# ChaissonLab/LRA

Hardware: AMD Instinct MI355X
Metric: aligned Gbp/s, 30 kb ONT vs GRCh38 (MapRead_lowacc end to end incl. SAM text), per job (higher is better)
Workload: dtype int32

## Files before the change

### lra_amd/csrc/indel_refine.hip

```cpp
#include "common.h"
#include "scan.h"
#include <algorithm>
#include <stdlib.h>

int lra_aog_launch_device(lra_ctx* ctx, int n, const char* d_qseq, const char* d_tseq, const uint64_t* d_q_off,
                          const int32_t* d_q_len, const uint64_t* d_t_off, const int32_t* d_t_len, const int32_t* d_k,
                          int m, int mm, int indel, int32_t* d_score, int32_t* d_nblocks, int32_t* d_blocks,
                          const uint64_t* d_block_off, int32_t* d_status);

namespace {

constexpr int BAD = -999999999;
constexpr int NEG = -2000000000;
enum { C_DIAG = 0, C_LEFT = 1, C_DOWN = 2, C_BOUND = 3, C_DELCLOSE = 4, C_INSCLOSE = 5, C_DONE = 6 };

__device__ __forceinline__ void wave_sync() {
  __builtin_amdgcn_fence(__ATOMIC_RELEASE, "workgroup");
  __builtin_amdgcn_wave_barrier();
  __builtin_amdgcn_fence(__ATOMIC_ACQUIRE, "workgroup");
}

__device__ __forceinline__ void wave_sync_lds() {
  __builtin_amdgcn_fence(__ATOMIC_RELEASE, "wavefront");
  __builtin_amdgcn_wave_barrier();
// ... 283 lines not shown
        }
    }
    if (st.btGap > st.bqGap) {
      for (int ti = 0; ti < st.btGap; ti++) {
        if (tOff >= tLen) { status |= 1; break; }
        const int e = (int)min(qEnd - 1, q + k);
        RG(ringS, tOff) = (int)max(q - k, qStart); RG(ringE, tOff) = e;
        if (e < eMin) eMin = e;
        if (sHi < tOff) sHi = tOff;
        tOff++;
        flush(tOff - k);
      }
    }
    bq = nq2; bt = nt2; bl = nl2;
  }
  if (lastChunk) for (long r = max(0L, tOff - k + 1); r < tLen; r++) flush(r);
#undef RG
  if (!multi) { if (tOff != tLen) status |= 1; B.s_status[s] = status; }
}

__global__ void __launch_bounds__(64) ir_band_scan(BandArgs B) {
  const uint64_t s = blockIdx.x;
  const int lane = threadIdx.x;
  if (B.s_kind[s] != 0) { if (lane == 0) { B.s_cells[s] = 0; B.s_status[s] = 0; B.s_width[s] = 0; B.s_tmpcap[s] = 0; } return; }
  int status = B.s_status[s];
  const long tLen = (long)B.s_rows[s];
  Row* rows = B.rows + B.s_row_off[s];
  unsigned long long cells = 0;
  int width = 0;
  if (!status && tLen > 0) {
    int run = 0x7fffffff;
    for (long base = ((tLen - 1) / 64) * 64; base >= 0; base -= 64) {
      const long r = base + lane;
      const int own = (r < tLen) ? rows[r].S : 0x7fffffff;
      int v = own;
      for (int d = 1; d < 64; d <<= 1) { int o = __shfl_down(v, d); if (lane + d < 64) v = min(v, o); }
      v = min(v, run);
      if (r < tLen && v != own) rows[r].S = v;
      run = __shfl(v, 0);
    }
    const int a = B.s_aln[s];
    const unsigned char* tb = (const unsigned char*)B.tseq + B.t_off[a] + B.s_tStart[s];
    int runE = -0x7fffffff;
    for (long base = 0; base < tLen; base += 64) {
      const long r = base + lane;
      Row w; w.S = 0; w.E = -0x7fffffff; w.C = 0; w.T = 0;
      if (r < tLen) w = rows[r];
      int e = w.E;
      for (int d = 1; d < 64; d <<= 1) { int o = __shfl_up(e, d); if (lane >= d) e = max(e, o); }
      e = max(e, runE);
      runE = __shfl(e, 63);
      int len = (r < tLen) ? e - w.S + 1 : 0;
      if (r < tLen) {
        if (len < 1 || w.S < 0) status |= 1;
        else if (len > MAXW) status |= 4;
        width = max(width, len);
      }
      const unsigned long long l = (unsigned long long)max(len, 0);
      unsigned long long inc = l;
      for (int d = 1; d < 64; d <<= 1) { unsigned long long o = __shfl_up(inc, d); if (lane >= d) inc += o; }
      if (r < tLen) { w.E = e; w.C = (unsigned int)(cells + inc - l); w.T = tb[r]; rows[r] = w; }
      cells += __shfl(inc, 63);
    }
    for (int o = 32; o > 0; o >>= 1) { status |= __shfl_xor(status, o); width = max(width, __shfl_xor(width, o)); }
  }
  if (lane == 0) {
    B.s_cells[s] = status ? 0 : cells;
    B.s_status[s] = status;
    B.s_width[s] = status ? 0 : width;
    B.s_tmpcap[s] = status ? 0 : (uint64_t)(tLen + ((long)B.s_qEnd[s] - B.s_qStart[s]) + 2);
  }
}

constexpr int FILL_BINS = 128;
template <bool EMIT>
__global__ void ir_classify(uint64_t n_seg, const int32_t* __restrict__ s_kind, const int32_t* __restrict__ s_status, const int32_t* __restrict__ s_width,
                            const uint64_t* __restrict__ s_rows, int* bins, uint32_t* list) {
  const uint64_t s = (uint64_t)blockIdx.x * blockDim.x + threadIdx.x;
  const int lane = threadIdx.x & 63;
  int bin = -1;
  if (s < n_seg && s_kind[s] == 0 && s_status[s] == 0) {
    const int w = s_width[s];
    const uint32_t r = (uint32_t)min((unsigned long long)s_rows[s], 0x7fffffffULL);
    bin = (w <= 16 ? 0 : w <= 32 ? 1 : w <= 64 ? 2 : 3) * 32 + (r ? __clz(r) : 31);
  }
  const unsigned long long below = (lane == 0) ? 0ULL : (~0ULL >> (64 - lane));
  unsigned long long todo = __ballot(bin >= 0);
  while (todo) {
    const int leader = __ffsll((long long)todo) - 1;
    const int b = __shfl(bin, leader);
    const unsigned long long m = __ballot(bin == b);
    int base = 0;
    if (lane == leader) base = atomicAdd(&bins[b], __popcll(m));
    base = __shfl(base, leader);
    if (EMIT && bin == b) list[base + __popcll(m & below)] = (uint32_t)s;
    todo &= ~m;
  }
}

struct FillArgs {
  uint64_t n_seg;
  const int32_t* s_aln; const uint64_t* s_rows; const uint64_t* s_row_off; const uint64_t* s_cell_off;
  const Row* rows;
  const char* qseq; const uint64_t* q_off; const int32_t* q_len;
  int match, mismatch, g;
  unsigned char* path;
  const uint32_t* list; int* cursor;
};

__device__ __forceinline__ bool is_bound(long row, int c, int len) { return c == len - 1 || (row > 0 && c == 0); }

__device__ __forceinline__ int shr1(int x, int fill) { return __builtin_amdgcn_update_dpp(fill, x, 0x138, 0xf, 0xf, false); }
template <int G>
__device__ __forceinline__ int scan_max(int w) {
  w = max(w, __builtin_amdgcn_update_dpp(NEG, w, 0x111, 0xf, 0xf, false));
  w = max(w, __builtin_amdgcn_update_dpp(NEG, w, 0x112, 0xf, 0xf, false));
  w = max(w, __builtin_amdgcn_update_dpp(NEG, w, 0x114, 0xf, 0xf, false));
  w = max(w, __builtin_amdgcn_update_dpp(NEG, w, 0x118, 0xf, 0xf, false));
  if (G >= 32) w = max(w, __builtin_amdgcn_update_dpp(NEG, w, 0x142, 0xa, 0xf, false));
  if (G >= 64) w = max(w, __builtin_amdgcn_update_dpp(NEG, w, 0x143, 0xc, 0xf, false));
  return w;
}

template <int G>
__global__ void __launch_bounds__(64) ir_fill(FillArgs F) {
  constexpr int GP = 64 / G;
  constexpr int CLS = (G == 16) ? 0 : (G == 32) ? 1 : 2;
  const int lane = threadIdx.x;
  const int c = lane % G, gbase = lane - c;
  const int g = F.g, go = 2 * F.g + 1;
  const long listEnd = F.cursor[4 + CLS];
  const uint32_t* list = F.list;
  long ti = -1, tLen = 0;
  const Row* rows = nullptr; const unsigned char* qb = nullptr; unsigned char* P = nullptr;
  long chunkBase = 0, qLast = 0;
  Row chunk; chunk.S = chunk.E = chunk.T = 0; chunk.C = 0;
  int W0 = 0, qlo = 0, qhi = 0, qnext = 0;
  int prevM = BAD, prevD = BAD, prevS = 0, prevLen = 0;
  bool done = false;
  auto ldq = [&](long idx) -> int { return qb[idx < qLast ? idx : qLast]; };
  while (true) {
    if (!done && ti < 0) {
      long x = 0;
      if (c == 0) x = atomicAdd(&F.cursor[CLS], 1);
      x = __shfl(x, gbase);
      if (x < listEnd) {
        const uint64_t s = list[x];
        const int a = F.s_aln[s];
        tLen = (long)F.s_rows[s];
        rows = F.rows + F.s_row_off[s];
        qb = (const unsigned char*)F.qseq + F.q_off[a];
        qLast = (long)F.q_len[a] - 1;
        P = F.path + F.s_cell_off[s];
        ti = 0; chunkBase = 0;
        if (c < tLen) chunk = rows[c];
        W0 = rows[0].S;
        qlo = ldq((long)W0 + c); qhi = ldq((long)W0 + G + c); qnext = ldq((long)W0 + 2 * G + c);
      } else done = true;
    }
    if (__ballot(!done) == 0ULL) break;
    if (!done && ti - chunkBase == G) { chunkBase = ti; if (ti + c < tLen) chunk = rows[ti + c]; }
    const int src = gbase + (int)((ti - chunkBase) & (G - 1));
    const int S = __shfl(chunk.S, src), E = __shfl(chunk.E, src), tch = __shfl(chunk.T, src);
    const unsigned int C = __shfl(chunk.C, src);
    while (!done && S - W0 >= G) { W0 += G; qlo = qhi; qhi = qnext; qnext = ldq((long)W0 + 2 * G + c); }
    const int j = S - W0 + c;
    const int q1 = __shfl(qlo, gbase + (j & (G - 1))), q2 = __shfl(qhi, gbase + (j & (G - 1)));
    const int qch = (j < G) ? q1 : q2;
    const int len = E - S + 1;
    const bool lastRow = (ti == tLen - 1);
    const int off = S - prevS;
    const bool interior = c >= 1 && (lastRow ? c <= len - 1 : c <= len - 2);
    const int srcA = c + off, srcD = srcA - 1;
    const bool aboveIn = srcA <= prevLen - 1;
    const int aM = __shfl(prevM, gbase + (srcA & (G - 1))), aD = __shfl(prevD, gbase + (srcA & (G - 1)));
    const int dM = shr1(aM, BAD);
    const bool okA = aboveIn && !is_bound(ti - 1, srcA, prevLen);
    const bool okD = aboveIn && srcD >= 0 && !is_bound(ti - 1, srcD, prevLen);
    const int dOpen = okA ? aM + go : BAD, dExt = okA ? aD : BAD;
    const int Dv = max(dOpen, dExt);
    const int delOpen = (Dv == dOpen) ? 1 : 0;
    const int mS = okD ? dM + (tch == qch ? F.match : F.mismatch) : BAD;
    const int dS = okA ? aM + g : BAD;
    const int V = interior ? max(mS, max(dS, Dv)) : NEG;
    const int W = scan_max<G>(V);
    int Wm1 = shr1(W, NEG), Vm1 = shr1(V, NEG);
    if (c == 0) { Wm1 = NEG; Vm1 = NEG; }
    const int Iv = max(BAD, go + Wm1);
    int M = max(max(BAD, V), max(Vm1 + g, go + Wm1));
    if (!interior) M = BAD;
    int Mleft = shr1(M, BAD);
    if (c <= 1) Mleft = BAD;
    const int iOpen = Mleft + go;
    const int insOpen = (Iv == iOpen) ? 1 : 0;
    const int iS = Mleft + g;
    int code;
    if (!interior) code = C_BOUND;
    else if (M == mS) code = C_DIAG;
    else if (M == iS) code = C_LEFT;
    else if (M == dS) code = C_DOWN;
    else if (M == Dv) code = C_DELCLOSE;
    else code = C_INSCLOSE;
    int outM = M, outD = interior ? Dv : BAD;
    unsigned char outB = (unsigned char)(code | (delOpen << 3) | (insOpen << 4));
    if (ti == 0) {
      const bool last0 = (c == len - 1) && (tLen > 1);
      outM = last0 ? BAD : (c == 0 ? 0 : c * g);
      outD = BAD;
      outB = (unsigned char)(last0 ? C_BOUND : (c == 0 ? C_DONE : C_LEFT));
    }
    if (!done) {
      if (c < len) P[C + c] = outB;
      prevM = outM; prevD = outD; prevS = S; prevLen = len;
      ti++;
      if (ti == tLen) ti = -1;
    }
  }
}


__global__ void __launch_bounds__(64) ir_fill_wide(FillArgs F) {
  __shared__ int sM[2][MAXW + 64], sD[2][MAXW + 64];
  const int lane = threadIdx.x;
  const int g = F.g, go = 2 * F.g + 1;
  const long listEnd = F.cursor[4 + 3];
  while (true) {
    long x = 0;
    if (lane == 0) x = atomicAdd(&F.cursor[3], 1);
    x = (long)(((unsigned long long)(unsigned)__builtin_amdgcn_readfirstlane((int)((unsigned long long)x >> 32)) << 32) | (unsigned)__builtin_amdgcn_readfirstlane((int)(x & 0xffffffffL)));
    if (x >= listEnd) break;
    const uint64_t s = F.list[x];
    const int a = F.s_aln[s];
    const long tLen = (long)F.s_rows[s];
    const Row* rows = F.rows + F.s_row_off[s];
    const unsigned char* qb = (const unsigned char*)F.qseq + F.q_off[a];
    const long qLast = (long)F.q_len[a] - 1;
    unsigned char* P = F.path + F.s_cell_off[s];
    int prevS = 0, prevLen = 0;
    for (long ti = 0; ti < tLen; ti++) {
      const Row rw = rows[ti];
      const int S = rw.S, len = rw.E - rw.S + 1, tch = rw.T;
      const unsigned int C = rw.C;
      const bool lastRow = (ti == tLen - 1);
      const int off = S - prevS;
      const int cur = (int)(ti & 1), prv = cur ^ 1;
      int carryW = NEG, carryV = NEG, carryM = BAD;
      for (int base = 0; base < len; base += 64) {
        const int c = base + lane;
        int outM, outD; unsigned char outB;
        if (ti == 0) {
          const bool last0 = (c == len - 1) && (tLen > 1);
          outM = last0 ? BAD : (c == 0 ? 0 : c * g);
          outD = BAD;
          outB = (unsigned char)(last0 ? C_BOUND : (c == 0 ? C_DONE : C_LEFT));
        } else {
          const long qi = (long)S + c;
          const int qch = qb[qi < qLast ? qi : qLast];
          const bool interior = c >= 1 && (lastRow ? c <= len - 1 : c <= len - 2);
          const int srcA = c + off, srcD = srcA - 1;
          const bool aboveIn = srcA <= prevLen - 1;
          const bool inA = srcA >= 0 && srcA < prevLen, inD = srcD >= 0 && srcD < prevLen;
          const int aM = inA ? sM[prv][srcA] : BAD, aD = inA ? sD[prv][srcA] : BAD;
          const int dM = inD ? sM[prv][srcD] : BAD;
          const bool okA = aboveIn && !is_bound(ti - 1, srcA, prevLen);
          const bool okD = aboveIn && srcD >= 0 && !is_bound(ti - 1, srcD, prevLen);
          const int dOpen = okA ? aM + go : BAD, dExt = okA ? aD : BAD;
          const int Dv = max(dOpen, dExt);
          const int delOpen = (Dv == dOpen) ? 1 : 0;
          const int mS = okD ? dM + (tch == qch ? F.match : F.mismatch) : BAD;
          const int dS = okA ? aM + g : BAD;
          const int V = interior ? max(mS, max(dS, Dv)) : NEG;
          const int W = max(scan_max<64>(V), carryW);
          int Wm1 = shr1(W, NEG), Vm1 = shr1(V, NEG);
          if (lane == 0) { Wm1 = carryW; Vm1 = carryV; }
          if (c == 0) { Wm1 = NEG; Vm1 = NEG; }
          const int Iv = max(BAD, go + Wm1);
          int M = max(max(BAD, V), max(Vm1 + g, go + Wm1));
          if (!interior) M = BAD;
          int Mleft = shr1(M, BAD);
          if (lane == 0) Mleft = carryM;
          if (c <= 1) Mleft = BAD;
          const int iOpen = Mleft + go;
          const int insOpen = (Iv == iOpen) ? 1 : 0;
          const int iS = Mleft + g;
          int code;
          if (!interior) code = C_BOUND;
          else if (M == mS) code = C_DIAG;
          else if (M == iS) code = C_LEFT;
          else if (M == dS) code = C_DOWN;
          else if (M == Dv) code = C_DELCLOSE;
          else code = C_INSCLOSE;
          outM = M; outD = interior ? Dv : BAD;
          outB = (unsigned char)(code | (delOpen << 3) | (insOpen << 4));
          carryW = __shfl(W, 63); carryV = __shfl(V, 63); carryM = __shfl(M, 63);
        }
        if (c < len) { P[C + c] = outB; sM[cur][c] = outM; sD[cur][c] = outD; }
      }
      wave_sync_lds();
      prevS = S; prevLen = len;
    }
  }
}

__global__ void __launch_bounds__(64) ir_fill_16x2(FillArgs F) {
  constexpr int G = 16;
  const int lane = threadIdx.x;
  const int c = lane % G, gbase = lane - c;
  const int g = F.g, go = 2 * F.g + 1;
  const long listEnd = F.cursor[4 + 1];
  const uint32_t* list = F.list;
  long ti = -1, tLen = 0;
  const Row* rows = nullptr; const unsigned char* qb = nullptr; unsigned char* P = nullptr;
  long chunkBase = 0, qLast = 0;
  Row chunk; chunk.S = chunk.E = chunk.T = 0; chunk.C = 0;
  int W0 = 0, q0 = 0, q1 = 0, q2 = 0, q3 = 0;
  int pM[2] = {BAD, BAD}, pD[2] = {BAD, BAD}, prevS = 0, prevLen = 0;
  bool done = false;
  auto ldq = [&](long idx) -> int { return qb[idx < qLast ? idx : qLast]; };
  while (true) {
    if (!done && ti < 0) {
      long x = 0;
      if (c == 0) x = atomicAdd(&F.cursor[1], 1);
      x = __shfl(x, gbase);
      if (x < listEnd) {
        const uint64_t s = list[x];
        const int a = F.s_aln[s];
        tLen = (long)F.s_rows[s];
        rows = F.rows + F.s_row_off[s];
        qb = (const unsigned char*)F.qseq + F.q_off[a];
        qLast = (long)F.q_len[a] - 1;
        P = F.path + F.s_cell_off[s];
        ti = 0; chunkBase = 0;
        if (c < tLen) chunk = rows[c];
        W0 = rows[0].S;
        q0 = ldq((long)W0 + c); q1 = ldq((long)W0 + G + c); q2 = ldq((long)W0 + 2 * G + c); q3 = ldq((long)W0 + 3 * G + c);
      } else done = true;
    }
    if (__ballot(!done) == 0ULL) break;
    if (!done && ti - chunkBase == G) { chunkBase = ti; if (ti + c < tLen) chunk = rows[ti + c]; }
    const int src = gbase + (int)((ti - chunkBase) & (G - 1));
    const int S = __shfl(chunk.S, src), E = __shfl(chunk.E, src), tch = __shfl(chunk.T, src);
    const unsigned int C = __shfl(chunk.C, src);
    while (!done && S - W0 >= G) { W0 += G; q0 = q1; q1 = q2; q2 = q3; q3 = ldq((long)W0 + 3 * G + c); }
    const int len = E - S + 1;
    const bool lastRow = (ti == tLen - 1);
    const int off = S - prevS;
    int nM[2] = {BAD, BAD}, nD[2] = {BAD, BAD};
    int carryW = NEG, carryV = NEG, carryM = BAD;
    const int np = (!done && len > G) ? 2 : 1;
    for (int p = 0; p < np; p++) {
      const int cc = c + G * p;
      const int j = S - W0 + cc;
      const int l = gbase + (j & (G - 1));
      const int qa = __shfl(q0, l), qbb = __shfl(q1, l), qc = __shfl(q2, l), qd = __shfl(q3, l);
      const int qch = (j < G) ? qa : (j < 2 * G) ? qbb : (j < 3 * G) ? qc : qd;
      const bool interior = cc >= 1 && (lastRow ? cc <= len - 1 : cc <= len - 2);
      const int srcA = cc + off, srcD = srcA - 1;
      const bool aboveIn = srcA <= prevLen - 1;
      const int la = gbase + (srcA & (G - 1)), ld = gbase + (srcD & (G - 1));
      const int a0 = __shfl(pM[0], la), a1 = __shfl(pM[1], la), b0 = __shfl(pD[0], la), b1 = __shfl(pD[1], la);
      const int d0 = __shfl(pM[0], ld), d1 = __shfl(pM[1], ld);
      const int aM = (srcA & G) ? a1 : a0, aD = (srcA & G) ? b1 : b0;
      const int dM = (srcD & G) ? d1 : d0;
      const bool okA = aboveIn && !is_bound(ti - 1, srcA, prevLen);
      const bool okD = aboveIn && srcD >= 0 && !is_bound(ti - 1, srcD, prevLen);
      const int dOpen = okA ? aM + go : BAD, dExt = okA ? aD : BAD;
      const int Dv = max(dOpen, dExt);
      const int delOpen = (Dv == dOpen) ? 1 : 0;
      const int mS = okD ? dM + (tch == qch ? F.match : F.mismatch) : BAD;
      const int dS = okA ? aM + g : BAD;
      const int V = interior ? max(mS, max(dS, Dv)) : NEG;
      const int W = max(scan_max<G>(V), carryW);
      int Wm1 = shr1(W, NEG), Vm1 = shr1(V, NEG);
      if (c == 0) { Wm1 = carryW; Vm1 = carryV; }
      const int Iv = max(BAD, go + Wm1);
      int M = max(max(BAD, V), max(Vm1 + g, go + Wm1));
      if (!interior) M = BAD;
      int Mleft = shr1(M, BAD);
      if (c == 0) Mleft = carryM;
      if (cc <= 1) Mleft = BAD;
      const int iOpen = Mleft + go;
      const int insOpen = (Iv == iOpen) ? 1 : 0;
      const int iS = Mleft + g;
      int code;
      if (!interior) code = C_BOUND;
      else if (M == mS) code = C_DIAG;
      else if (M == iS) code = C_LEFT;
      else if (M == dS) code = C_DOWN;
      else if (M == Dv) code = C_DELCLOSE;
      else code = C_INSCLOSE;
      int outM = M, outD = interior ? Dv : BAD;
      unsigned char outB = (unsigned char)(code | (delOpen << 3) | (insOpen << 4));
      if (ti == 0) {
        const bool last0 = (cc == len - 1) && (tLen > 1);
        outM = last0 ? BAD : (cc == 0 ? 0 : cc * g);
        outD = BAD;
        outB = (unsigned char)(last0 ? C_BOUND : (cc == 0 ? C_DONE : C_LEFT));
      }
      if (!done && cc < len) P[C + cc] = outB;
      nM[p] = outM; nD[p] = outD;
      carryW = __shfl(W, gbase + G - 1); carryV = __shfl(V, gbase + G - 1); carryM = __shfl(M, gbase + G - 1);
    }
    if (!done) {
      pM[0] = nM[0]; pM[1] = nM[1]; pD[0] = nD[0]; pD[1] = nD[1]; prevS = S; prevLen = len;
      ti++;
      if (ti == tLen) ti = -1;
    }
  }
}

struct TraceArgs {
  uint64_t n_seg;
  const int32_t* s_kind; const int32_t* s_tStart; const uint64_t* s_rows; const uint64_t* s_row_off;
  const uint64_t* s_cells; const uint64_t* s_cell_off; int32_t* s_status;
  const Row* rows;
  const unsigned char* path;
  uint32_t* s_nblk;
  const uint64_t* s_tmp_off; int32_t* tmp_blocks;
};

constexpr int TW_ROWS = 128, TW_PATH = 4096;
__global__ void __launch_bounds__(64) ir_trace_wave(TraceArgs T) {
  __shared__ Row s_rows[TW_ROWS];
  __shared__ __attribute__((aligned(16))) unsigned char s_path[TW_PATH + 16];
  const int lane = threadIdx.x;
  const uint64_t s = blockIdx.x;
  if (s >= T.n_seg) return;
  if (T.s_kind[s] != 0) return;
  if (T.s_status[s] != 0) { if (lane == 0) T.s_nblk[s] = 0; return; }
  const long tLen = (long)T.s_rows[s];
  const Row* rows = T.rows + T.s_row_off[s];
  const unsigned char* P = T.path + T.s_cell_off[s];
  int32_t* ob = T.tmp_blocks + 3 * T.s_tmp_off[s];
  const long cap = (long)(T.s_tmp_off[s + 1] - T.s_tmp_off[s]);
  long ti = tLen - 1;
  long rBase = 0, wLo = 1, wHi = 0; unsigned pBase = 0;
  auto stage = [&](long at) {
    wave_sync();
    wHi = at; rBase = max(0L, at - TW_ROWS + 1);
    for (long x = lane; x <= at - rBase; x += 64) s_rows[x] = rows[rBase + x];
    wave_sync();
    const Row last = s_rows[at - rBase];
    const unsigned end = last.C + (unsigned)max(last.E - last.S + 1, 0);
    long lo = rBase, hi = at;
    while (lo < hi) { const long mid = (lo + hi) >> 1; if (end - s_rows[mid - rBase].C <= (unsigned)TW_PATH) hi = mid; else lo = mid + 1; }
    wLo = lo; pBase = s_rows[lo - rBase].C;
    const unsigned nbytes = min(end - pBase, (unsigned)TW_PATH);
    const unsigned char* start = P + pBase;
    const unsigned delta = (unsigned)((uintptr_t)start & 15);
    const uint4* a16 = (const uint4*)(start - delta);
    const unsigned full = (delta + nbytes) >> 4;
    for (unsigned x = lane; x < full; x += 64) ((uint4*)s_path)[x] = a16[x];
    for (unsigned x = (full << 4) + lane; x < delta + nbytes; x += 64) s_path[x] = (start - delta)[x];
    pBase -= delta;
    wave_sync();
  };
  stage(ti);
  Row rw = s_rows[ti - rBase];
  int qa = rw.E;
  int mat = 0;
  int bad = 0;
  long nblk = 0;
  long q = (long)rw.E + 1, t = (long)T.s_tStart[s] + tLen;
  int curKind = -1, pending = 0;
  long dlen = 0;
  long steps = 0;
  const long step_cap = 4 * (long)T.s_cells[s] + 64;
  auto emit_block = [&]() {
    if (nblk < cap) { if (lane == 0) { ob[3 * nblk] = (int)q; ob[3 * nblk + 1] = (int)t; ob[3 * nblk + 2] = (int)dlen; } } else bad = 1;
    nblk++;
  };
  auto op = [&](int kind, long times) {
    if (kind != curKind) {
      if (curKind == -1 && kind == 0) { pending = 1; dlen = 0; }
      if (kind != 0) {
        if (pending) emit_block();
        pending = 1; dlen = 0;
      }
      curKind = kind;
    }
    if (kind == 0) { dlen += times; q -= times; t -= times; }
    else if (kind == 1) q -= times;
    else t -= times;
  };
  while (true) {
    if (ti < wLo || ti > wHi) stage(ti);
    rw = s_rows[ti - rBase];
    if (mat == 0) {
      const long tl = ti - lane;
      bool fast = false;
      if (tl >= wLo && tl >= 1) {
        const Row r = s_rows[tl - rBase];
        const int c = (qa - lane) - r.S;
        if (c >= 0 && c <= r.E - r.S) fast = (s_path[r.C - pBase + (unsigned)c] & 7) == C_DIAG;
      }
      const unsigned long long nf = ~__ballot(fast);
      const int f = nf ? __ffsll((long long)nf) - 1 : 64;
      if (f > 0) {
        steps += f;
        if (steps > step_cap) { bad = 1; break; }
        op(0, f); ti -= f; qa -= f;
        continue;
      }
    }
    const int c = qa - rw.S;
    if (c < 0 || c > rw.E - rw.S) { bad = 1; break; }
    if (ti == 0 && c == 0) break;
    if (++steps > step_cap) { bad = 1; break; }
    const unsigned char pb = s_path[rw.C - pBase + (unsigned)c];
    long nti = ti;
    if (mat == 0) {
      const int code = pb & 7;
      if (code == C_DELCLOSE) mat = 1;
      else if (code == C_INSCLOSE) mat = 2;
      else if (code == C_DIAG) { op(0, 1); nti = ti - 1; qa--; }
      else if (code == C_LEFT) { op(1, 1); qa--; }
      else if (code == C_DOWN) { op(2, 1); nti = ti - 1; }
      else { bad = 1; break; }
    } else if (mat == 1) {
      op(2, 1);
      mat = ((pb >> 3) & 1) ? 0 : 1;
      nti = ti - 1;
    } else {
      op(1, 1);
      mat = ((pb >> 4) & 1) ? 0 : 2;
      qa--;
    }
    if (nti != ti) {
      if (nti < 0) { bad = 1; break; }
      ti = nti;
    }
  }
  if (!bad) {
    op(0, 1);
    if (pending) emit_block();
  }
  if (lane == 0) {
    if (bad) T.s_status[s] |= 2;
    T.s_nblk[s] = bad ? 0 : (uint32_t)nblk;
  }
}

struct GatherArgs {
  uint64_t n_item;
  const int32_t* i_kind; const int32_t* i_data; const int32_t* i_aln; const uint64_t* i_out_off;
  const uint64_t* seg_off;
  const int32_t* s_kind; const int32_t* s_qStart; const int32_t* s_tStart; const uint32_t* s_aog_idx;
  const int32_t* aog_blocks; const uint64_t* aog_block_off; const int32_t* aog_nblocks;
  const int32_t* tmp_blocks; const uint64_t* s_tmp_off; const uint32_t* s_nblk;
  int32_t* out_blocks;
};

__global__ void ir_item_counts(uint64_t n_item, const int32_t* i_kind, const int32_t* i_data, const int32_t* i_aln, const uint64_t* seg_off,
                               const int32_t* s_kind, const uint32_t* s_nblk, const uint32_t* s_aog_idx, const int32_t* aog_nblocks,
                               uint32_t* i_count) {
  uint64_t i = (uint64_t)blockIdx.x * blockDim.x + threadIdx.x;
  if (i >= n_item) return;
  if (i_kind[i] == 0) { i_count[i] = 1; return; }
  uint64_t s = seg_off[i_aln[i]] + (uint64_t)i_data[3 * i];
  i_count[i] = (s_kind[s] == 0) ? s_nblk[s] : (uint32_t)aog_nblocks[s_aog_idx[s]];
}

__global__ void __launch_bounds__(64) ir_gather(GatherArgs G) {
  const int lane = threadIdx.x;
  for (uint64_t i = blockIdx.x; i < G.n_item; i += gridDim.x) {
    int32_t* out = G.out_blocks + 3 * G.i_out_off[i];
    if (G.i_kind[i] == 0) {
      if (lane < 3) out[lane] = G.i_data[3 * i + lane];
      continue;
    }
    uint64_t s = G.seg_off[G.i_aln[i]] + (uint64_t)G.i_data[3 * i];
    if (G.s_kind[s] == 0) {
      const int32_t* src = G.tmp_blocks + 3 * G.s_tmp_off[s];
      const int n = (int)G.s_nblk[s];
      for (int x = lane; x < n; x += 64) {
        const int y = n - 1 - x;
        out[3 * x] = src[3 * y]; out[3 * x + 1] = src[3 * y + 1]; out[3 * x + 2] = src[3 * y + 2];
      }
      continue;
    }
    const uint32_t p = G.s_aog_idx[s];
    const int32_t* src = G.aog_blocks + 3 * G.aog_block_off[p];
    const int n = G.aog_nblocks[p];
    const int qs = G.s_qStart[s], ts = G.s_tStart[s];
    for (int x = lane; x < n; x += 64) {
      out[3 * x] = src[3 * x] + qs; out[3 * x + 1] = src[3 * x + 1] + ts; out[3 * x + 2] = src[3 * x + 2];
    }
  }
}

__global__ void ir_finalize_offsets(int n_aln, uint64_t n_item, const uint64_t* item_off, const uint64_t* i_out_off, const int32_t* i_kind,
                                    const int32_t* i_data, const int32_t* i_aln, const uint64_t* seg_off, uint64_t* s_out_off,
                                    uint64_t* out_block_off) {
  uint64_t i = (uint64_t)blockIdx.x * blockDim.x + threadIdx.x;
  if (i <= (uint64_t)n_aln) out_block_off[i] = i_out_off[i < (uint64_t)n_aln ? item_off[i] : n_item];
  if (i < n_item && i_kind[i] == 1) s_out_off[seg_off[i_aln[i]] + (uint64_t)i_data[3 * i]] = i_out_off[i];
}

__global__ void ir_aln_status(int n_aln, const uint64_t* seg_off, const int32_t* s_kind, const int32_t* s_status, const uint32_t* s_aog_idx,
                              const int32_t* p_status, int32_t* a_status) {
  int a = blockIdx.x * blockDim.x + threadIdx.x;
  if (a >= n_aln) return;
  int st = 0;
  for (uint64_t s = seg_off[a]; s < seg_off[a + 1]; s++) {
    if (s_kind[s] == 0) { int x = s_status[s]; if (x & 1) st |= LRA_ST_OOB_SLOT; if (x & 2) st |= LRA_ST_NO_TERMINATION; if (x & 4) st |= LRA_ST_RANGE; }
    else st |= p_status[s_aog_idx[s]];
  }
  a_status[a] = st;
}

__global__ void ir_item_aln(int n_aln, const uint64_t* item_off, int32_t* i_aln) {
  int a = blockIdx.x * blockDim.x + threadIdx.x;
  if (a >= n_aln) return;
  for (uint64_t i = item_off[a]; i < item_off[a + 1]; i++) i_aln[i] = a;
}

__global__ void ir_aog_setup(uint64_t n_seg, const int32_t* s_kind, const int32_t* s_aln, const uint64_t* s_aog_off ,
                             const int32_t* s_qStart, const int32_t* s_tStart, const int32_t* s_qEnd, const int32_t* s_tEnd,
                             const uint64_t* q_off, const uint64_t* t_off, int k, uint32_t* s_aog_idx, uint64_t* p_q_off, int32_t* p_q_len,
                             uint64_t* p_t_off, int32_t* p_t_len, int32_t* p_k, uint32_t* p_cap) {
  uint64_t s = (uint64_t)blockIdx.x * blockDim.x + threadIdx.x;
  if (s >= n_seg) return;
  if (s_kind[s] != 1) { s_aog_idx[s] = 0; return; }
  uint32_t p = (uint32_t)s_aog_off[s];
  s_aog_idx[s] = p;
  int a = s_aln[s];
  p_q_off[p] = q_off[a] + (uint64_t)s_qStart[s]; p_q_len[p] = s_qEnd[s] - s_qStart[s];
  p_t_off[p] = t_off[a] + (uint64_t)s_tStart[s]; p_t_len[p] = s_tEnd[s] - s_tStart[s];
  p_k[p] = k;
  p_cap[p] = (uint32_t)(min(p_q_len[p], p_t_len[p]) + 1);
}


struct Arena {
  char* base; size_t cap, used;
  template <typename T> T* get(size_t n) {
    size_t bytes = (n * sizeof(T) + 255) & ~(size_t)255;
    if (used + bytes > cap) return nullptr;
    T* p = (T*)(base + used);
    used += bytes;
    return p;
  }
};

}

template <typename CT>
static void scan(lra_ctx* ctx, long n, const CT* c, uint64_t* off) {
  (void)lra_exclusive_scan<CT>(ctx, n, c, off);
}

static int d2h(lra_ctx* ctx, void* dst, const void* src, size_t bytes) {
  LRA_HIP_CHECK(ctx, hipMemcpyAsync(dst, src, bytes, hipMemcpyDeviceToHost, ctx->stream));
  LRA_HIP_CHECK(ctx, hipStreamSynchronize(ctx->stream));
  return LRA_OK;
}

extern "C" int lra_indel_refine_batch(lra_ctx* ctx, int n_aln, const int32_t* d_blocks_in, const uint64_t* d_block_off, uint64_t n_blocks_in,
                                      const char* d_qseq, const uint64_t* d_q_off, const int32_t* d_q_len, const char* d_tseq,
                                      const uint64_t* d_t_off, const int64_t* d_t_len, int refine_band, int match, int mismatch,
                                      int indel, int end_align, lra_refine_result* out) {
  if (!ctx || !out || n_aln < 0) return LRA_ERR_INVALID;
  if (refine_band < 2 || refine_band > 64) return lra_set_err(ctx, LRA_ERR_INVALID, "refine_band must be 2..64");
  if (indel >= 0) return lra_set_err(ctx, LRA_ERR_INVALID, "indel score must be negative");
  memset(out, 0, sizeof(*out));
  if (n_aln == 0) return LRA_OK;
  LRA_HIP_CHECK(ctx, hipSetDevice(ctx->device));
  hipStream_t st = ctx->stream;
  const size_t nA = (size_t)n_aln, nBk = (size_t)n_blocks_in + 2 * nA;
  const size_t perAln = ((nA * 4 + 255) & ~(size_t)255) * 3 + (((nA + 1) * 8 + 255) & ~(size_t)255) * 3;
  char* baseP = (char*)lra_ensure(ctx, 70, perAln + 4096);
  if (!baseP) return LRA_ERR_NOMEM;
  Arena ap{baseP, perAln + 4096, 0};
  IRArgs A;
  memset(&A, 0, sizeof A);
  A.n_aln = n_aln; A.blocks_in = d_blocks_in; A.block_off = d_block_off;
  A.qseq = d_qseq; A.q_off = d_q_off; A.q_len = d_q_len; A.tseq = d_tseq; A.t_off = d_t_off; A.t_len = d_t_len;
  A.k = refine_band; A.match = match; A.mismatch = mismatch; A.indel = indel; A.endAlign = end_align;
  A.a_nseg = ap.get<uint32_t>(nA); A.a_nitem = ap.get<uint32_t>(nA); A.a_status = ap.get<int32_t>(nA);
  uint64_t* seg_off = ap.get<uint64_t>(nA + 1); uint64_t* item_off = ap.get<uint64_t>(nA + 1); uint64_t* out_block_off = ap.get<uint64_t>(nA + 1);
  if (!out_block_off) return lra_set_err(ctx, LRA_ERR_NOMEM, "arena accounting");
  A.seg_off = seg_off; A.item_off = item_off;
  const int nbA = (n_aln + SEG_LANES - 1) / SEG_LANES;
  lra_time_begin(ctx, "ir_segment");
  hipLaunchKernelGGL(ir_segment<false>, dim3(nbA), dim3(64), 0, st, A);
  lra_time_end(ctx);
  scan(ctx, (long)n_aln, A.a_nseg, seg_off);
  scan(ctx, (long)n_aln, A.a_nitem, item_off);
  uint64_t n_seg = 0, n_item = 0;
  if (d2h(ctx, &n_seg, seg_off + n_aln, 8) || d2h(ctx, &n_item, item_off + n_aln, 8)) return LRA_ERR_HIP;
  const size_t capSeg = (size_t)n_seg + 1, capItem = (size_t)n_item + 1;
  size_t needA = 0;
  auto add = [&](size_t n, size_t sz) { needA += ((n * sz + 255) & ~(size_t)255); };
  add(3 * nBk, 4);
  for (int i = 0; i < 8; i++) add(capSeg, 4);
  add(3 * capSeg, 4); add(capSeg, 4); add(capSeg, 8); add(capSeg, 4);
  add(capSeg + 1, 8); add(capSeg + 1, 8); add(capSeg, 8); add(capSeg + 1, 8); add(capSeg, 4);
  add(capSeg, 4); add(capSeg, 4); add(capSeg, 8); add(capSeg + 1, 8); add(capSeg, 4); add(capSeg + 1, 8);
  add(capSeg, 4); add(FILL_BINS + 8, 4);
  add(capItem, 4); add(3 * capItem, 4); add(capItem, 4); add(capItem, 4); add(capItem + 1, 8);
  add(capSeg, 8); add(capSeg, 4); add(capSeg, 8); add(capSeg, 4); add(capSeg, 4); add(capSeg, 4); add(capSeg + 1, 8);
  add(capSeg, 4); add(capSeg, 4); add(capSeg, 4);
  add(capSeg, 4); add(capSeg + 1, 8);
  char* baseA = (char*)lra_scratch(ctx, 2, needA + 4096);
  if (!baseA) return LRA_ERR_NOMEM;
  Arena ar{baseA, needA + 4096, 0};
  A.ab = ar.get<int32_t>(3 * nBk);
  A.s_aln = ar.get<int32_t>(capSeg); A.s_kind = ar.get<int32_t>(capSeg); A.s_qStart = ar.get<int32_t>(capSeg); A.s_tStart = ar.get<int32_t>(capSeg);
  A.s_qEnd = ar.get<int32_t>(capSeg); A.s_tEnd = ar.get<int32_t>(capSeg); A.s_b0 = ar.get<int32_t>(capSeg); A.s_b1 = ar.get<int32_t>(capSeg);
  A.s_first = ar.get<int32_t>(3 * capSeg); A.s_lastLen = ar.get<int32_t>(capSeg); A.s_rows = ar.get<uint64_t>(capSeg); A.s_isAog = ar.get<uint32_t>(capSeg);
  uint64_t* s_row_off = ar.get<uint64_t>(capSeg + 1); uint64_t* s_aog_off = ar.get<uint64_t>(capSeg + 1);
  uint64_t* s_cells = ar.get<uint64_t>(capSeg); uint64_t* s_cell_off = ar.get<uint64_t>(capSeg + 1); int32_t* s_status = ar.get<int32_t>(capSeg);
  uint32_t* s_nblk = ar.get<uint32_t>(capSeg); int32_t* s_width = ar.get<int32_t>(capSeg); uint64_t* s_tmpcap = ar.get<uint64_t>(capSeg);
  uint64_t* s_tmp_off = ar.get<uint64_t>(capSeg + 1); uint32_t* s_aog_idx = ar.get<uint32_t>(capSeg); uint64_t* s_out_off = ar.get<uint64_t>(capSeg + 1);
  uint32_t* fill_lists = ar.get<uint32_t>(capSeg); int* fill_counts = ar.get<int>(FILL_BINS + 8);
  A.i_kind = ar.get<int32_t>(capItem); A.i_data = ar.get<int32_t>(3 * capItem);
  int32_t* i_aln = ar.get<int32_t>(capItem); uint32_t* i_count = ar.get<uint32_t>(capItem); uint64_t* i_out_off = ar.get<uint64_t>(capItem + 1);
  uint64_t* p_q_off = ar.get<uint64_t>(capSeg); int32_t* p_q_len = ar.get<int32_t>(capSeg); uint64_t* p_t_off = ar.get<uint64_t>(capSeg);
  int32_t* p_t_len = ar.get<int32_t>(capSeg); int32_t* p_k = ar.get<int32_t>(capSeg); uint32_t* p_cap = ar.get<uint32_t>(capSeg);
  uint64_t* p_block_off = ar.get<uint64_t>(capSeg + 1);
  int32_t* p_score = ar.get<int32_t>(capSeg); int32_t* p_nblocks = ar.get<int32_t>(capSeg); int32_t* p_status = ar.get<int32_t>(capSeg);
  uint32_t* s_nchunk = ar.get<uint32_t>(capSeg); uint64_t* chunk_off = ar.get<uint64_t>(capSeg + 1);
  if (!chunk_off) return lra_set_err(ctx, LRA_ERR_NOMEM, "arena accounting");
  lra_time_begin(ctx, "ir_segment");
  hipLaunchKernelGGL(ir_segment<true>, dim3(nbA), dim3(64), 0, st, A);
  lra_time_end(ctx);
  hipLaunchKernelGGL(ir_item_aln, dim3((n_aln + 255) / 256), dim3(256), 0, st, n_aln, item_off, i_aln);
  uint64_t n_rows = 0, n_aog = 0, n_cells = 0;
  const int32_t* tmp_blocks = nullptr;
  if (n_seg) {
    scan(ctx, (long)n_seg, A.s_rows, s_row_off);
    scan(ctx, (long)n_seg, A.s_isAog, s_aog_off);
    if (d2h(ctx, &n_rows, s_row_off + n_seg, 8) || d2h(ctx, &n_aog, s_aog_off + n_seg, 8)) return LRA_ERR_HIP;
    Row* rows = (Row*)lra_ensure(ctx, 0, (n_rows + 1) * sizeof(Row));
    if (!rows) return LRA_ERR_NOMEM;
    BandArgs B;
    B.n_seg = n_seg; B.s_aln = A.s_aln; B.s_kind = A.s_kind; B.s_qStart = A.s_qStart; B.s_qEnd = A.s_qEnd; B.s_tStart = A.s_tStart;
    B.s_b0 = A.s_b0; B.s_b1 = A.s_b1; B.s_first = A.s_first; B.s_lastLen = A.s_lastLen; B.s_rows = A.s_rows; B.s_row_off = s_row_off;
    B.ab = A.ab; B.block_off = d_block_off; B.tseq = d_tseq; B.t_off = d_t_off; B.k = refine_band; B.rows = rows;
    B.s_cells = s_cells; B.s_status = s_status; B.s_width = s_width; B.s_tmpcap = s_tmpcap;
    const unsigned gridL = (unsigned)((n_seg + 63) / 64);
    const unsigned gridS = (unsigned)((n_seg + 255) / 256);
    lra_time_begin(ctx, "ir_band");
    B.s_nchunk = s_nchunk; B.chunk_off = chunk_off; B.n_task = 0; B.task_seg = nullptr; B.chunkT = nullptr; B.chunkQ = nullptr;
    hipLaunchKernelGGL(ir_band_nchunk, dim3(gridS), dim3(256), 0, st, B);
    scan(ctx, (long)n_seg, s_nchunk, chunk_off);
    uint64_t n_task = 0;
    if (d2h(ctx, &n_task, chunk_off + n_seg, 8)) return LRA_ERR_HIP;
    uint32_t* task_seg = (uint32_t*)lra_ensure(ctx, 54, (n_task + 1) * 4);
    int32_t* chunk_tq = (int32_t*)lra_ensure(ctx, 55, (n_task + 1) * 8);
    if (!task_seg || !chunk_tq) return LRA_ERR_NOMEM;
    B.n_task = n_task; B.task_seg = task_seg; B.chunkT = chunk_tq; B.chunkQ = chunk_tq + n_task + 1;
    hipLaunchKernelGGL(ir_band_tasks, dim3(gridS), dim3(256), 0, st, B);
    hipLaunchKernelGGL(ir_band_prep, dim3((unsigned)n_seg), dim3(64), 0, st, B);
    if (n_task) {
      const unsigned gridT = (unsigned)((n_task + 63) / 64);
      if (refine_band <= 8) hipLaunchKernelGGL(ir_band_chunk<16>, dim3(gridT), dim3(64), 0, st, B);
      else if (refine_band <= 32) hipLaunchKernelGGL(ir_band_chunk<64>, dim3(gridT), dim3(64), 0, st, B);
      else hipLaunchKernelGGL(ir_band_chunk<128>, dim3(gridT), dim3(64), 0, st, B);
    }
    hipLaunchKernelGGL(ir_band_scan, dim3((unsigned)n_seg), dim3(64), 0, st, B);
    lra_time_end(ctx);
    scan(ctx, (long)n_seg, s_cells, s_cell_off);
    scan(ctx, (long)n_seg, s_tmpcap, s_tmp_off);
    uint64_t n_tmp = 0;
    if (d2h(ctx, &n_cells, s_cell_off + n_seg, 8) || d2h(ctx, &n_tmp, s_tmp_off + n_seg, 8)) return LRA_ERR_HIP;
    const size_t pathBytes = (n_cells + 256 + 255) & ~(size_t)255;
    unsigned char* path = (unsigned char*)lra_ensure(ctx, 12, pathBytes + (n_tmp + 1) * 12 + 256);
    if (!path) return LRA_ERR_NOMEM;
    int32_t* tmpb = (int32_t*)(path + pathBytes);
    tmp_blocks = tmpb;
    int h_bins[FILL_BINS], h_start[FILL_BINS], h_cursor[8] = {0, 0, 0, 0, 0, 0, 0, 0};
    LRA_HIP_CHECK(ctx, hipMemsetAsync(fill_counts, 0, FILL_BINS * 4, st));
    hipLaunchKernelGGL(ir_classify<false>, dim3((unsigned)((n_seg + 255) / 256)), dim3(256), 0, st, n_seg, A.s_kind, s_status, s_width, A.s_rows, fill_counts, fill_lists);
    if (d2h(ctx, h_bins, fill_counts, FILL_BINS * 4)) return LRA_ERR_HIP;
    { int run = 0; for (int b = 0; b < FILL_BINS; b++) { h_start[b] = run; run += h_bins[b]; if ((b & 31) == 0) h_cursor[b / 32] = h_start[b]; if ((b & 31) == 31) h_cursor[4 + b / 32] = run; } }
    LRA_HIP_CHECK(ctx, hipMemcpyAsync(fill_counts, h_start, FILL_BINS * 4, hipMemcpyHostToDevice, st));
    hipLaunchKernelGGL(ir_classify<true>, dim3((unsigned)((n_seg + 255) / 256)), dim3(256), 0, st, n_seg, A.s_kind, s_status, s_width, A.s_rows, fill_counts, fill_lists);
    int* fill_cursor = fill_counts + FILL_BINS;
    LRA_HIP_CHECK(ctx, hipMemcpyAsync(fill_cursor, h_cursor, 32, hipMemcpyHostToDevice, st));
    FillArgs F;
    F.n_seg = n_seg; F.s_aln = A.s_aln; F.s_rows = A.s_rows; F.s_row_off = s_row_off; F.s_cell_off = s_cell_off; F.rows = rows;
    F.qseq = d_qseq; F.q_off = d_q_off; F.q_len = d_q_len; F.match = match; F.mismatch = mismatch; F.g = indel; F.path = path;
    F.list = fill_lists; F.cursor = fill_cursor;
    const unsigned cap_grid = (unsigned)ctx->num_cu * 32;
    if (getenv("LRA_IR_DBG")) {
      const int hc[4] = {h_cursor[4] - h_cursor[0], h_cursor[5] - h_cursor[1], h_cursor[6] - h_cursor[2], h_cursor[7] - h_cursor[3]};
      fprintf(stderr, "[ir] n_seg %llu n_rows %llu n_cells %llu n_task %llu n_item %llu fill classes 16/32/64/wide: %d %d %d %d\n",
              (unsigned long long)n_seg, (unsigned long long)n_rows, (unsigned long long)n_cells, (unsigned long long)n_task,
              (unsigned long long)n_item, hc[0], hc[1], hc[2], hc[3]);
    }
    lra_time_begin(ctx, "ir_fill");
    const uint64_t n16 = (uint64_t)(h_cursor[4] - h_cursor[0]), n32 = (uint64_t)(h_cursor[5] - h_cursor[1]), n64 = (uint64_t)(h_cursor[6] - h_cursor[2]);
    const uint64_t nWide = (uint64_t)(h_cursor[7] - h_cursor[3]);
    if (n16) hipLaunchKernelGGL(ir_fill<16>, dim3((unsigned)std::min<uint64_t>((n16 + 3) / 4, cap_grid)), dim3(64), 0, lra_side_fork(ctx, 1), F);
    if (n64) hipLaunchKernelGGL(ir_fill<64>, dim3((unsigned)std::min<uint64_t>(n64, cap_grid)), dim3(64), 0, lra_side_fork(ctx, 2), F);
    if (nWide) hipLaunchKernelGGL(ir_fill_wide, dim3((unsigned)std::min<uint64_t>(nWide, cap_grid)), dim3(64), 0, lra_side_fork(ctx, 3), F);
    if (n32) hipLaunchKernelGGL(ir_fill_16x2, dim3((unsigned)std::min<uint64_t>((n32 + 3) / 4, cap_grid)), dim3(64), 0, st, F);
    if (n16) lra_side_join(ctx, 1);
    if (n64) lra_side_join(ctx, 2);
    if (nWide) lra_side_join(ctx, 3);
    lra_time_end(ctx);
    TraceArgs T;
    T.n_seg = n_seg; T.s_kind = A.s_kind; T.s_tStart = A.s_tStart; T.s_rows = A.s_rows; T.s_row_off = s_row_off;
    T.s_cells = s_cells; T.s_cell_off = s_cell_off; T.s_status = s_status; T.rows = rows; T.path = path;
    T.s_nblk = s_nblk; T.s_tmp_off = s_tmp_off; T.tmp_blocks = tmpb;
    lra_time_begin(ctx, "ir_trace");
    hipLaunchKernelGGL(ir_trace_wave, dim3((unsigned)n_seg), dim3(64), 0, st, T);
    lra_time_end(ctx);
    if (n_aog) {
      hipLaunchKernelGGL(ir_aog_setup, dim3((unsigned)((n_seg + 255) / 256)), dim3(256), 0, st, n_seg, A.s_kind, A.s_aln, s_aog_off, A.s_qStart,
                         A.s_tStart, A.s_qEnd, A.s_tEnd, d_q_off, d_t_off, refine_band, s_aog_idx, p_q_off, p_q_len, p_t_off, p_t_len, p_k, p_cap);
      scan(ctx, (long)n_aog, p_cap, p_block_off);
      uint64_t aog_cap = 0;
      if (d2h(ctx, &aog_cap, p_block_off + n_aog, 8)) return LRA_ERR_HIP;
      if (aog_cap * 12 + 64 > ctx->aux_bytes) {
        if (ctx->aux) (void)hipFree(ctx->aux);
        ctx->aux = nullptr; ctx->aux_bytes = 0;
        size_t want = aog_cap * 12 + aog_cap * 3 + 4096;
        if (hipMalloc(&ctx->aux, want) != hipSuccess) return lra_set_err(ctx, LRA_ERR_NOMEM, "aog block buffer");
        ctx->aux_bytes = want;
      }
      int rc = lra_aog_launch_device(ctx, (int)n_aog, d_qseq, d_tseq, p_q_off, p_q_len, p_t_off, p_t_len, p_k, match, mismatch, indel, p_score,
                                     p_nblocks, (int32_t*)ctx->aux, p_block_off, p_status);
      if (rc) return rc;
    }
  }
  hipLaunchKernelGGL(ir_item_counts, dim3((unsigned)((n_item + 255) / 256)), dim3(256), 0, st, n_item, A.i_kind, A.i_data, i_aln, seg_off, A.s_kind,
                     s_nblk, s_aog_idx, p_nblocks, i_count);
  scan(ctx, (long)n_item, i_count, i_out_off);
  uint64_t n_out = 0;
  if (d2h(ctx, &n_out, i_out_off + n_item, 8)) return LRA_ERR_HIP;
  if ((n_out + 1) * 12 > ctx->out_bytes) {
    if (ctx->out_buf) (void)hipFree(ctx->out_buf);
    ctx->out_buf = nullptr; ctx->out_bytes = 0;
    size_t want = (n_out + 1) * 12 + (n_out + 1) * 3 + 4096;
    if (hipMalloc(&ctx->out_buf, want) != hipSuccess) return lra_set_err(ctx, LRA_ERR_NOMEM, "refined block buffer");
    ctx->out_bytes = want;
  }
  int32_t* out_blocks = (int32_t*)ctx->out_buf;
  hipLaunchKernelGGL(ir_finalize_offsets, dim3((unsigned)((std::max<uint64_t>(n_item, nA + 1) + 255) / 256)), dim3(256), 0, st, n_aln, n_item, item_off,
                     i_out_off, A.i_kind, A.i_data, i_aln, seg_off, s_out_off, out_block_off);
  GatherArgs G;
  G.n_item = n_item; G.i_kind = A.i_kind; G.i_data = A.i_data; G.i_aln = i_aln; G.i_out_off = i_out_off; G.seg_off = seg_off;
  G.s_kind = A.s_kind; G.s_qStart = A.s_qStart; G.s_tStart = A.s_tStart; G.s_aog_idx = s_aog_idx;
  G.aog_blocks = (const int32_t*)ctx->aux; G.aog_block_off = p_block_off; G.aog_nblocks = p_nblocks;
  G.tmp_blocks = tmp_blocks; G.s_tmp_off = s_tmp_off; G.s_nblk = s_nblk; G.out_blocks = out_blocks;
  lra_time_begin(ctx, "ir_gather");
  if (n_item) hipLaunchKernelGGL(ir_gather, dim3((unsigned)std::min<uint64_t>(n_item, 65535 * 4)), dim3(64), 0, st, G);
  lra_time_end(ctx);
  hipLaunchKernelGGL(ir_aln_status, dim3((n_aln + 255) / 256), dim3(256), 0, st, n_aln, seg_off, A.s_kind, s_status, s_aog_idx, p_status, A.a_status);
  LRA_HIP_CHECK(ctx, hipGetLastError());
  LRA_HIP_CHECK(ctx, hipStreamSynchronize(st));
  out->n_aln = n_aln; out->n_blocks = n_out; out->n_segments = n_seg; out->n_cells = n_cells; out->n_rows = n_rows; out->n_aog = n_aog;
  out->d_block_off = out_block_off; out->d_blocks = out_blocks; out->d_status = A.a_status;
  return LRA_OK;
}
```

Baseline: 1.064.

## Use column-aligned ring layout with DPP rotations in narrow indel-refine fill kernels

Rewrites the 16-lane-group fill kernel as a template (1 or 2 column passes) that keeps cells at fixed absolute-column lanes modulo 16. Neighbor accesses then become DPP row rotations instead of general shuffles, and the prefix max becomes a ring scan gated by distance. Row metadata is staged through LDS rather than four shuffles per row. The query window advances in 16-aligned blocks. The new kernel also replaces the previous width-16 ir_fill kernel, which adds correctness risk around wraparound and carry handling at the head lane.

```diff
diff --git a/lra_amd/csrc/indel_refine.hip b/lra_amd/csrc/indel_refine.hip
--- a/lra_amd/csrc/indel_refine.hip
+++ b/lra_amd/csrc/indel_refine.hip
@@ -609,25 +609,40 @@
   }
 }
 
-__global__ void __launch_bounds__(64) ir_fill_16x2(FillArgs F) {
+template <int N>
+__device__ __forceinline__ int ror(int x) { return __builtin_amdgcn_update_dpp(0, x, 0x120 + N, 0xf, 0xf, true); }
+__device__ __forceinline__ int pin(int x) { asm volatile("" : "+v"(x)); return x; }
+__device__ __forceinline__ int ring_scan_max(int w, int d) {
+  { const int t = pin(max(w, ror<1>(w))); w = (d >= 1) ? t : w; }
+  { const int t = pin(max(w, ror<2>(w))); w = (d >= 2) ? t : w; }
+  { const int t = pin(max(w, ror<4>(w))); w = (d >= 4) ? t : w; }
+  { const int t = pin(max(w, ror<8>(w))); w = (d >= 8) ? t : w; }
+  return w;
+}
+template <int NP>
+__global__ void __launch_bounds__(64) ir_fill_cols(FillArgs F) {
   constexpr int G = 16;
+  constexpr int CLS = NP - 1;
   const int lane = threadIdx.x;
   const int c = lane % G, gbase = lane - c;
   const int g = F.g, go = 2 * F.g + 1;
-  const long listEnd = F.cursor[4 + 1];
+  const long listEnd = F.cursor[4 + CLS];
   const uint32_t* list = F.list;
   long ti = -1, tLen = 0;
   const Row* rows = nullptr; const unsigned char* qb = nullptr; unsigned char* P = nullptr;
-  long chunkBase = 0, qLast = 0;
+  long qLast = 0;
+  __shared__ Row s_chunk[64];
+  long chunkBase = 0;
   Row chunk; chunk.S = chunk.E = chunk.T = 0; chunk.C = 0;
-  int W0 = 0, q0 = 0, q1 = 0, q2 = 0, q3 = 0;
-  int pM[2] = {BAD, BAD}, pD[2] = {BAD, BAD}, prevS = 0, prevLen = 0;
+  int K0 = 0, q0 = 0, q1 = 0, q2 = 0, q3 = 0;
+  int pM[NP], pD[NP], prevS = 0, prevLen = 0;
+  for (int p = 0; p < NP; p++) { pM[p] = BAD; pD[p] = BAD; }
   bool done = false;
   auto ldq = [&](long idx) -> int { return qb[idx < qLast ? idx : qLast]; };
   while (true) {
     if (!done && ti < 0) {
       long x = 0;
-      if (c == 0) x = atomicAdd(&F.cursor[1], 1);
+      if (c == 0) x = atomicAdd(&F.cursor[CLS], 1);
       x = __shfl(x, gbase);
       if (x < listEnd) {
         const uint64_t s = list[x];
@@ -637,38 +652,51 @@
         qb = (const unsigned char*)F.qseq + F.q_off[a];
         qLast = (long)F.q_len[a] - 1;
         P = F.path + F.s_cell_off[s];
-        ti = 0; chunkBase = 0;
+        ti = 0; chunkBase = -G;
         if (c < tLen) chunk = rows[c];
-        W0 = rows[0].S;
-        q0 = ldq((long)W0 + c); q1 = ldq((long)W0 + G + c); q2 = ldq((long)W0 + 2 * G + c); q3 = ldq((long)W0 + 3 * G + c);
+        K0 = rows[0].S >> 4;
+        const long b = 16L * K0 + c;
+        q0 = ldq(b); q1 = ldq(b + G); q2 = ldq(b + 2 * G); q3 = ldq(b + 3 * G);
       } else done = true;
     }
     if (__ballot(!done) == 0ULL) break;
-    if (!done && ti - chunkBase == G) { chunkBase = ti; if (ti + c < tLen) chunk = rows[ti + c]; }
-    const int src = gbase + (int)((ti - chunkBase) & (G - 1));
-    const int S = __shfl(chunk.S, src), E = __shfl(chunk.E, src), tch = __shfl(chunk.T, src);
-    const unsigned int C = __shfl(chunk.C, src);
-    while (!done && S - W0 >= G) { W0 += G; q0 = q1; q1 = q2; q2 = q3; q3 = ldq((long)W0 + 3 * G + c); }
+    if (!done && ti - chunkBase == G) {
+      chunkBase = ti;
+      s_chunk[lane] = chunk;
+      wave_sync_lds();
+      if (ti + G + c < tLen) chunk = rows[ti + G + c];
+    }
+    const Row rw = s_chunk[gbase + (int)((ti - chunkBase) & (G - 1))];
+    const int S = rw.S, E = rw.E, tch = rw.T;
+    const unsigned int C = rw.C;
+    if (!done && (S >> 4) != K0) {
+      const int adv = (S >> 4) - K0;
+      K0 = S >> 4;
+      const long b = 16L * K0 + c;
+      if (adv == 1) { q0 = q1; q1 = q2; q2 = q3; }
+      else { q0 = ldq(b); q1 = ldq(b + G); q2 = ldq(b + 2 * G); }
+      q3 = ldq(b + 3 * G);
+    }
     const int len = E - S + 1;
     const bool lastRow = (ti == tLen - 1);
     const int off = S - prevS;
-    int nM[2] = {BAD, BAD}, nD[2] = {BAD, BAD};
-    int carryW = NEG, carryV = NEG, carryM = BAD;
-    const int np = (!done && len > G) ? 2 : 1;
-    for (int p = 0; p < np; p++) {
-      const int cc = c + G * p;
-      const int j = S - W0 + cc;
-      const int l = gbase + (j & (G - 1));
-      const int qa = __shfl(q0, l), qbb = __shfl(q1, l), qc = __shfl(q2, l), qd = __shfl(q3, l);
-      const int qch = (j < G) ? qa : (j < 2 * G) ? qbb : (j < 3 * G) ? qc : qd;
+    const int d = (c - S) & (G - 1);
+    const bool head = (d == 0);
+    const bool lo = c >= (S & (G - 1));
+    int nM[NP], nD[NP];
+    for (int p = 0; p < NP; p++) { nM[p] = BAD; nD[p] = BAD; }
+    int cW = NEG, cV = NEG, cM = BAD, cA = BAD;
+    for (int p = 0; p < NP; p++) {
+      if (p == 1 && len <= G) break;
+      const int cc = d + G * p;
+      const int qch = (p == 0) ? (lo ? q0 : q1) : (lo ? q1 : q2);
       const bool interior = cc >= 1 && (lastRow ? cc <= len - 1 : cc <= len - 2);
       const int srcA = cc + off, srcD = srcA - 1;
       const bool aboveIn = srcA <= prevLen - 1;
-      const int la = gbase + (srcA & (G - 1)), ld = gbase + (srcD & (G - 1));
-      const int a0 = __shfl(pM[0], la), a1 = __shfl(pM[1], la), b0 = __shfl(pD[0], la), b1 = __shfl(pD[1], la);
-      const int d0 = __shfl(pM[0], ld), d1 = __shfl(pM[1], ld);
-      const int aM = (srcA & G) ? a1 : a0, aD = (srcA & G) ? b1 : b0;
-      const int dM = (srcD & G) ? d1 : d0;
+      const int aM = (NP > 1 && srcA >= G) ? pM[NP - 1] : pM[0];
+      const int aD = (NP > 1 && srcA >= G) ? pD[NP - 1] : pD[0];
+      const int rA = pin(ror<1>(aM));
+      const int dM = (p == 1 && head) ? cA : rA;
       const bool okA = aboveIn && !is_bound(ti - 1, srcA, prevLen);
       const bool okD = aboveIn && srcD >= 0 && !is_bound(ti - 1, srcD, prevLen);
       const int dOpen = okA ? aM + go : BAD, dExt = okA ? aD : BAD;
@@ -677,14 +705,14 @@
       const int mS = okD ? dM + (tch == qch ? F.match : F.mismatch) : BAD;
       const int dS = okA ? aM + g : BAD;
       const int V = interior ? max(mS, max(dS, Dv)) : NEG;
-      const int W = max(scan_max<G>(V), carryW);
-      int Wm1 = shr1(W, NEG), Vm1 = shr1(V, NEG);
-      if (c == 0) { Wm1 = carryW; Vm1 = carryV; }
+      const int W = ring_scan_max((p == 1 && head) ? max(V, cW) : V, d);
+      const int rW = pin(ror<1>(W)), rV = pin(ror<1>(V));
+      const int Wm1 = head ? cW : rW, Vm1 = head ? cV : rV;
       const int Iv = max(BAD, go + Wm1);
       int M = max(max(BAD, V), max(Vm1 + g, go + Wm1));
       if (!interior) M = BAD;
-      int Mleft = shr1(M, BAD);
-      if (c == 0) Mleft = carryM;
+      const int rM = pin(ror<1>(M));
+      int Mleft = head ? cM : rM;
       if (cc <= 1) Mleft = BAD;
       const int iOpen = Mleft + go;
       const int insOpen = (Iv == iOpen) ? 1 : 0;
@@ -706,10 +734,11 @@
       }
       if (!done && cc < len) P[C + cc] = outB;
       nM[p] = outM; nD[p] = outD;
-      carryW = __shfl(W, gbase + G - 1); carryV = __shfl(V, gbase + G - 1); carryM = __shfl(M, gbase + G - 1);
+      if (NP > 1 && p == 0) { cW = rW; cV = rV; cM = rM; cA = rA; }
     }
     if (!done) {
-      pM[0] = nM[0]; pM[1] = nM[1]; pD[0] = nD[0]; pD[1] = nD[1]; prevS = S; prevLen = len;
+      for (int p = 0; p < NP; p++) { pM[p] = nM[p]; pD[p] = nD[p]; }
+      prevS = S; prevLen = len;
       ti++;
       if (ti == tLen) ti = -1;
     }
@@ -1100,10 +1129,10 @@
     lra_time_begin(ctx, "ir_fill");
     const uint64_t n16 = (uint64_t)(h_cursor[4] - h_cursor[0]), n32 = (uint64_t)(h_cursor[5] - h_cursor[1]), n64 = (uint64_t)(h_cursor[6] - h_cursor[2]);
     const uint64_t nWide = (uint64_t)(h_cursor[7] - h_cursor[3]);
-    if (n16) hipLaunchKernelGGL(ir_fill<16>, dim3((unsigned)std::min<uint64_t>((n16 + 3) / 4, cap_grid)), dim3(64), 0, lra_side_fork(ctx, 1), F);
+    if (n16) hipLaunchKernelGGL(ir_fill_cols<1>, dim3((unsigned)std::min<uint64_t>((n16 + 3) / 4, cap_grid)), dim3(64), 0, lra_side_fork(ctx, 1), F);
     if (n64) hipLaunchKernelGGL(ir_fill<64>, dim3((unsigned)std::min<uint64_t>(n64, cap_grid)), dim3(64), 0, lra_side_fork(ctx, 2), F);
     if (nWide) hipLaunchKernelGGL(ir_fill_wide, dim3((unsigned)std::min<uint64_t>(nWide, cap_grid)), dim3(64), 0, lra_side_fork(ctx, 3), F);
-    if (n32) hipLaunchKernelGGL(ir_fill_16x2, dim3((unsigned)std::min<uint64_t>((n32 + 3) / 4, cap_grid)), dim3(64), 0, st, F);
+    if (n32) hipLaunchKernelGGL(ir_fill_cols<2>, dim3((unsigned)std::min<uint64_t>((n32 + 3) / 4, cap_grid)), dim3(64), 0, st, F);
     if (n16) lra_side_join(ctx, 1);
     if (n64) lra_side_join(ctx, 2);
     if (nWide) lra_side_join(ctx, 3);
```

Result: faster. 1.090 (median of 6 runs) (+2.4%).
